# MingSun-Tse/Efficient-NeRF

Hardware: AMD Instinct MI355X
Metric: rays/sec at 800x800 (R2L W256D88) (higher is better)
Workload: dtype f16+bf6 (1 fp16 MFMA pass + both hi/lo correction terms on the block-scaled MFMA in OCP bf6 (e3m2) at 4x the fp16 rate, fp32 accumulate)

## Files before the change

efficient-nerf_amd/csrc/gen/head_gen.py:

```python
#!/usr/bin/env python3
import argparse
import os
import sys

import numpy as np

import isa
from isa import (Ins, State, Filler, vr, ar, vreg, areg, sreg, mfma32_16, mfma32_6, ds_read_b128, ds_read_b64, waitcnt_lgkm,
                 waitcnt_vm, barrier, valu, v_max0, v_accr, v_cvt_pk_f16, v_resid16, v_cvt_pk32_bf6, s_nop, salu, f_to_bf6,
                 pack6, layer_exponent, weight_exps, f32_bits, check_hazards_stream, model_cycles, v_f32_op, v_fma_f32,
                 v_ldexp_f32, v_rndne_f32, v_sin_f32, v_max3_abs)

V_O, V_D, V_X, V_RH, V_RL = 0, 3, 6, 9, 12
V_BQ = 15
V_TT = 16
V_EP = 16
V_VAL = 48
V_EH = 80
V_E6 = 112
V_LO = 136
V_HI = 152
V_A6 = 184
V_L0, V_L1, V_L8A, V_L8B, V_AUX, V_LOFF, V_LANE, V_ST = 196, 197, 198, 199, 200, 201, 202, 203
V_SBA, V_SBL, V_CVA, V_CVL = 204, 205, 206, 207
V_SC = 208
N_VGPR_CLOBBER = 210
V_HMAX = 210
NHI = 8
A_X = 0
N_AGPR_CLOBBER = 128

S_W, S_XOUT, S_WAVE, S_NEG1, S_M0SAVE = 40, 42, 44, 45, 46
S_G = 48
S_WPW = 50
S_C = 51
S_P2 = 54
N_SGPR_LO, N_SGPR_HI = 40, 64

NSLOT = 4
AUX_BYTES = 2048
AUX_SCALES = 1024
NPT = 16
NCH = 2 * NPT


def configure(fmt):
    global FMT, PIECES, CHUNK, PW, LDS_AUX, LDS_BYTES, STREAM_BYTES, ANCH_PER_RT, ANCH_PER_CHUNK, N_ANCH, NHI, NHL, V_HL, V_EL, NAME
    FMT = fmt
    PIECES = 32 if fmt == 'f16' else 28
    CHUNK = PIECES * 1024
    PW = PIECES // 4
    LDS_AUX = NSLOT * CHUNK
    LDS_BYTES = LDS_AUX + AUX_BYTES
    STREAM_BYTES = NCH * CHUNK
    ANCH_PER_RT = 12 if fmt == 'f16' else 6
    ANCH_PER_CHUNK = 4 * ANCH_PER_RT
    N_ANCH = NCH * ANCH_PER_CHUNK
    NHI = 6 if fmt == 'f16' else 8
    NHL, V_HL = 5, 176
    V_EL = 112
    NAME = 'r2l_headx' if fmt == 'f16' else 'r2l_head'


configure('bf6')
EMB_EXP = -1
RES_SHIFT = 12
INV2PI_HI = np.float32(0.15915494)
INV2PI_LO = np.float32(6.4206382e-09)
J_ORDER = [(0, 0), (1, 0)]


def X(u):
    return A_X + u * 16


def EH(b, s):
    return V_EH + b * 16 + s * 4


def E6(b, term):
    return V_E6 + b * 12 + term * 6


def EL(b, s):
    return V_EL + b * 16 + s * 4


def head_col(p, s, h, j):
    if s < 3:
        return (3 * p + s) * 21 + (10 if h else 0) + j
    if j < 6:
        return (3 * p + (j >> 1)) * 21 + (10 if h else 0) + 8 + (j & 1)
    if j == 6:
        return (3 * p + (2 if h else 0)) * 21 + 20
    return -1 if h else (3 * p + 1) * 21 + 20


def piece_hi(k, s):
    return k * 4 + s


def piece_a6(k, t):
    return 16 + k * 2 + t


def piece_a6b(k, t):
    return 24 + k, t * 512


def pack_head(W, b, act_scale=16.0, fmt='bf6'):
    configure(fmt)
    Ws = (W.astype(np.float64) * act_scale).astype(np.float32)
    hi = Ws.astype(np.float16)
    el, ew = weight_exps(layer_exponent(Ws))
    img = np.zeros(STREAM_BYTES, dtype=np.uint8)
    aux = np.zeros(AUX_BYTES // 4, dtype=np.uint32)
    aux[:256] = (b.astype(np.float64) * act_scale).astype(np.float32).view(np.uint32)
    for q in range(4):
        aux[AUX_SCALES // 4 + 4 * q] = 0x01010101 * (127 + el)
        aux[AUX_SCALES // 4 + 4 * q + 1] = 0x01010101 * (127 + ew)
    lanes = np.arange(64)
    h, r = lanes >> 5, lanes & 31
    for p in range(NPT):
        cols = np.array([[[head_col(p, s, hh, j) for j in range(8)] for s in range(4)] for hh in range(2)])
        for u in range(8):
            base = (2 * p + (u >> 2)) * CHUNK
            k = u & 3
            rows = 32 * u + r
            col = cols[h]
            wv = np.where(col >= 0, Ws[rows[:, None, None], np.maximum(col, 0)], 0).astype(np.float32)
            wh = np.where(col >= 0, hi[rows[:, None, None], np.maximum(col, 0)], 0).astype(np.float16)
            for s in range(4):
                o = base + piece_hi(k, s) * 1024
                img[o:o + 1024] = np.ascontiguousarray(wh[:, s, :]).view(np.uint8).reshape(-1)
            if FMT == 'f16':
                wl = (wv.astype(np.float64) - wh.astype(np.float64)).astype(np.float16)
                for s in range(4):
                    o = base + (16 + piece_hi(k, s)) * 1024
                    img[o:o + 1024] = np.ascontiguousarray(wl[:, s, :]).view(np.uint8).reshape(-1)
                continue
            w64, h64 = wv.reshape(64, 32).astype(np.float64), wh.reshape(64, 32).astype(np.float64)
            for t, v in enumerate((np.ldexp(w64 - h64, -el), np.ldexp(w64, -ew))):
                words = pack6(f_to_bf6(v))
                o = base + piece_a6(k, t) * 1024
                img[o:o + 1024] = np.ascontiguousarray(words[:, :4]).view(np.uint8).reshape(-1)
                pc, off = piece_a6b(k, t)
                o = base + pc * 1024 + off
                img[o:o + 512] = np.ascontiguousarray(words[:, 4:]).view(np.uint8).reshape(-1)
    return img, aux.view(np.uint8)


def zop(p):
    return ('s', 'z%d' % p)


def v_sel_half(dst, lo_src, hi_src):
    def emu(st):
        a = isa._f32(st, lo_src).view(np.uint32)
        b = isa._f32(st, hi_src).view(np.uint32)
        st.V[dst] = np.where(np.arange(64) >= 32, b, a)
    return valu('v_cndmask_b32 %s, %s, %s, vcc' % (vreg(dst), isa._opnd(lo_src), isa._opnd(hi_src)), isa._rd(lo_src, hi_src),
                vr(dst), emu)


def dma_piece(i, tag=''):
    voffr = V_L0 if i < 4 else V_LOFF
    imm = 1024 * (i & 3)
    text = 'global_load_lds_dwordx4 %s, %s offset:%d' % (vreg(voffr), sreg(S_G, 2), imm)

    def emu(st):
        copies = []
        g = st.S[S_G]
        for w in range(4):
            dw = (w - st.wave) * PW * 1024
            for l in range(64):
                src = g + int(st.V[voffr][l]) + dw + imm
                dst = st.m0 + dw + imm + l * 16
                assert 0 <= dst and dst + 16 <= LDS_AUX, dst
                assert 0 <= src and src + 16 <= len(st.img), src
                copies.append((dst, st.img[src:src + 16].copy()))
                st.lds_pending[dst:dst + 16] = True
        st.pend_dma.append(copies)
    return Ins(text, 'dma', rd=vr(voffr), emu=emu, cost=8, tag=tag)


def store_group(i, src):
    text = 'global_store_dwordx4 %s, %s, %s offset:%d' % (vreg(V_L0), vreg(src, 4), sreg(S_XOUT, 2), (i & 3) * 1024)

    def emu(st):
        st.xout[i] = st.V[src:src + 4].copy()
    return Ins(text, 'store', rd=vr(V_L0) + vr(src, 4), emu=emu, cost=4)


class HState(State):
    def __init__(self, wave, img, aux, z):
        State.__init__(self, wave, img, np.zeros((1, 1024), dtype=np.uint32), 0, LDS_BYTES)
        self.lds[LDS_AUX:LDS_AUX + len(aux)] = aux
        for p in range(NPT):
            self.S['z%d' % p] = float(z[p])
        self.xout = {}


def embed_ops(p):
    b = p & 1
    ops = []
    for c in range(3):
        ops.append(v_f32_op('mul', V_X + c, zop(p), ('v', V_D + c)))
    for c in range(3):
        ops.append(v_f32_op('add', V_X + c, ('v', V_O + c), ('v', V_X + c)))
    for c in range(3):
        ops.append(v_f32_op('mul', V_RH + c, ('s', S_C), ('v', V_X + c)))
    for c in range(3):
        ops.append(v_fma_f32(V_RL + c, ('v', V_X + c), ('s', S_C), ('v', V_RH + c), neg_c=True))
    for c in range(3):
        ops.append(v_fma_f32(V_RL + c, ('v', V_X + c), ('s', S_C + 1), ('v', V_RL + c)))
    vals = [(8 * c + l, c, l) for c in range(3) for l in range(8)] + [(24 + j, j >> 1, 8 + (j & 1)) for j in range(6)]
    for i0 in range(0, len(vals), 4):
        grp = vals[i0:i0 + 4]
        T = [V_TT + 3 * k for k in range(len(grp))]
        for k, (e, c, l) in enumerate(grp):
            ops.append(v_fma_f32(T[k], ('v', V_RH + c), ('s', S_P2 + l), ('v', V_BQ)))
        for k in range(len(grp)):
            ops.append(v_rndne_f32(T[k] + 1, ('v', T[k])))
        for k in range(len(grp)):
            ops.append(v_f32_op('sub', T[k], ('v', T[k]), ('v', T[k] + 1)))
        for k, (e, c, l) in enumerate(grp):
            ops.append(v_fma_f32(T[k], ('v', V_RL + c), ('s', S_P2 + l), ('v', T[k])))
        for k, (e, c, l) in enumerate(grp):
            ops.append(v_sin_f32(V_VAL + e, ('v', T[k])))
    ops.append(v_sel_half(V_VAL + 30, ('v', V_X + 0), ('v', V_X + 2)))
    ops.append(v_sel_half(V_VAL + 31, ('v', V_X + 1), 0.0))
    for i in range(16):
        ops.append(v_cvt_pk_f16(EH(b, 0) + i, V_VAL + 2 * i, V_VAL + 2 * i + 1))
    for half in range(2):
        for i in range(16):
            ops.append(v_resid16((EL(b, 0) if FMT == 'f16' else V_LO) + i, half, EH(b, 0) + i, half, V_VAL + 2 * i + half, S_NEG1))
    if FMT == 'f16':
        return ops
    ops.append(v_cvt_pk32_bf6(E6(b, 0), EH(b, 0), V_CVA))
    ops.append(v_cvt_pk32_bf6(E6(b, 1), V_LO, V_CVL))
    return ops




def anchor(ci, k, kind, sj):
    if FMT == 'f16':
        return ci * ANCH_PER_CHUNK + k * ANCH_PER_RT + 3 * sj + ('m16', 'mhl', 'mlh').index(kind)
    return ci * ANCH_PER_CHUNK + k * 6 + (sj if kind == 'm16' else 4 + sj)


def lds_addr(slot, byte_off, width):
    off = slot * CHUNK + byte_off
    lo, hi = (V_L0, V_L1) if width == 16 else (V_L8A, V_L8B)
    return (lo, off) if off < 65536 else (hi, off - 65536)


def chunk_issue_seq(cn):
    off = (cn % NCH) * CHUNK
    slot = cn % NSLOT
    seq = [salu('s_add_u32 %s, %s, %s' % (sreg(S_G), sreg(S_W), sreg(S_WPW)), lambda st: st.S.__setitem__(S_G, st.S[S_W] + st.S[S_WPW])),
           salu('s_addc_u32 %s, %s, 0' % (sreg(S_G + 1), sreg(S_W + 1)))]
    if off:
        seq += [salu('s_add_u32 %s, %s, 0x%x' % (sreg(S_G), sreg(S_G), off), lambda st: st.S.__setitem__(S_G, st.S[S_G] + off)),
                salu('s_addc_u32 %s, %s, 0' % (sreg(S_G + 1), sreg(S_G + 1)))]
    seq.append(salu('s_add_u32 m0, %s, 0x%x' % (sreg(S_WPW), slot * CHUNK), lambda st: setattr(st, 'm0', st.S[S_WPW] + slot * CHUNK)))
    seq.append(s_nop(0))
    for i in range(PW):
        if i == 4:
            seq.append(salu('s_add_u32 m0, m0, 0x1000', lambda st: setattr(st, 'm0', st.m0 + 4096)))
            seq.append(s_nop(0))
        seq.append(dma_piece(i, tag=('dma', cn, i)))
    return seq


class Opts:
    def __init__(self, **kw):
        self.rd_lead = 6
        self.rd_lead6 = 5
        self.cap = 7
        self.dma_gap = 1
        self.pair_waits = True
        self.fmt = 'bf6'
        self.__dict__.update(kw)


def build_fillers(opts):
    F = []
    n16, n6 = 0, 0
    last16, last6 = {}, {}
    HALF = ANCH_PER_CHUNK // 2
    for ci in range(NCH):
        for k in range(4):
            for s in range(4):
                a = anchor(ci, k, 'm16', s)
                prev = last16.get(n16 - NHI, -1)
                pc = piece_hi(k, s)
                bv, off = lds_addr(ci % NSLOT, pc * 1024, 16)
                cert = -1 if ci < 3 else (ci - 1) * ANCH_PER_CHUNK + HALF + 1
                F.append(Filler(ds_read_b128(V_HI + (n16 % NHI) * 4, bv, off, tag=('hi', ci, k, s)),
                                max(prev, a - opts.rd_lead, cert), a, ('rd',)))
                last16[n16] = anchor(ci, k, 'mhl', s) if FMT == 'f16' else a
                if FMT == 'f16':
                    al = anchor(ci, k, 'mlh', s)
                    bv, off = lds_addr(ci % NSLOT, (16 + pc) * 1024, 16)
                    F.append(Filler(ds_read_b128(V_HL + (n16 % NHL) * 4, bv, off, tag=('hl', ci, k, s)),
                                    max(last6.get(n16 - NHL, -1), al - opts.rd_lead, cert), al, ('rdl',)))
                    last6[n16] = al
                n16 += 1
            for t in range(2 if FMT != 'f16' else 0):
                a = anchor(ci, k, 'm6', t)
                prev = last6.get(n6 - 2, -1)
                cert = -1 if ci < 3 else (ci - 1) * ANCH_PER_CHUNK + HALF + 1
                e = max(prev, a - opts.rd_lead6, cert)
                bv, off = lds_addr(ci % NSLOT, piece_a6(k, t) * 1024, 16)
                F.append(Filler(ds_read_b128(V_A6 + (n6 & 1) * 6, bv, off, tag=('a6', ci, k, t, 0)), e, a, ('rd6',)))
                pc, po = piece_a6b(k, t)
                bv, off = lds_addr(ci % NSLOT, pc * 1024 + po, 8)
                F.append(Filler(ds_read_b64(V_A6 + (n6 & 1) * 6 + 4, bv, off, tag=('a6', ci, k, t, 1)), e, a, ('rd6',)))
                last6[n6] = a
                n6 += 1
    for p in range(NPT - 1):
        a0, a1 = 2 * p * ANCH_PER_CHUNK, (2 * p + 2) * ANCH_PER_CHUNK
        ops = embed_ops(p + 1)
        for i, ins in enumerate(ops):
            F.append(Filler(ins, a0 + (i * (a1 - a0 - 6)) // len(ops), a1 - 3, ('emb',)))
    for ci in range(NCH):
        ar = ci * ANCH_PER_CHUNK + HALF
        ch = ('dma',)
        F.append(Filler(waitcnt_vm(PW if ci >= 1 else 0), ar - 1, ar + 1, ch))
        F.append(Filler(barrier(), ar - 1, ar + 1, ch))
        k = 0
        for ins in chunk_issue_seq(ci + 3):
            if ins.kind != 'dma' and k == 0:
                F.append(Filler(ins, ar - 1, ar + 3, ch))
            else:
                F.append(Filler(ins, ar + 1 + opts.dma_gap * k, ar + ANCH_PER_CHUNK - 2, ch))
                if ins.kind == 'dma':
                    k += 1
    return F


class Sched:
    def __init__(self):
        self.out = []
        self.ds_issued = 0
        self.ds_done = 0
        self.ds_index = {}

    def emit(self, ins):
        self.out.append(ins)
        if ins.kind == 'ds':
            self.ds_index[ins.tag] = self.ds_issued
            self.ds_issued += 1

    def need(self, key, also=()):
        idx = self.ds_index[key]
        if idx < self.ds_done:
            return
        for k2 in also:
            if k2 in self.ds_index:
                idx = max(idx, self.ds_index[k2])
        self.emit(waitcnt_lgkm(self.ds_issued - idx - 1))
        self.ds_done = idx + 1


def schedule(opts):
    sch = Sched()
    fillers = build_fillers(opts)
    for i, f in enumerate(fillers):
        f.seq = i
    chains = {}
    for f in fillers:
        chains.setdefault(f.chain, []).append(f)
    for ch in chains.values():
        for i in range(len(ch) - 2, -1, -1):
            ch[i].deadline = min(ch[i].deadline, ch[i + 1].deadline)
    heads = {ch: 0 for ch in chains}

    def ready(pos):
        r = []
        for ch, lst in chains.items():
            i = heads[ch]
            if i < len(lst) and lst[i].earliest <= pos:
                r.append(lst[i])
        r.sort(key=lambda f: (f.deadline, f.seq))
        return r

    def issue(f):
        sch.emit(f.ins)
        heads[f.chain] += 1

    while True:
        r = ready(-1)
        if not r:
            break
        issue(r[0])
    n16 = n6 = 0
    for a in range(N_ANCH):
        while True:
            r = [f for f in ready(a - 1) if f.deadline <= a]
            if not r:
                break
            issue(r[0])
        ci, rem = divmod(a, ANCH_PER_CHUNK)
        k, j = divmod(rem, ANCH_PER_RT)
        p, u = ci >> 1, 4 * (ci & 1) + k
        b = p & 1
        if FMT == 'f16':
            sj, which = divmod(j, 3)
            if which == 0:
                sch.need(('hi', ci, k, sj))
                ins = mfma32_16('a', X(u), V_HI + (n16 % NHI) * 4, EH(b, sj), 'a', X(u), tag=('m16', ci, k, sj))
            elif which == 1:
                ins = mfma32_16('a', X(u), V_HI + (n16 % NHI) * 4, EL(b, sj), 'a', X(u), tag=('mhl', ci, k, sj))
            else:
                sch.need(('hl', ci, k, sj))
                ins = mfma32_16('a', X(u), V_HL + (n16 % NHL) * 4, EH(b, sj), 'a', X(u), tag=('mlh', ci, k, sj))
                n16 += 1
        elif j < 4:
            nxt = [('hi', ci, k, j + 1)] if j < 3 and opts.pair_waits else []
            sch.need(('hi', ci, k, j), nxt)
            ins = mfma32_16('a', X(u), V_HI + (n16 % NHI) * 4, EH(b, j), 'a', X(u), tag=('m16', ci, k, j))
            n16 += 1
        else:
            t = j - 4
            sch.need(('a6', ci, k, t, 1))
            ins = mfma32_6('a', X(u), V_A6 + (n6 & 1) * 6, E6(b, t), V_SC + t, V_SBA if t == 0 else V_SBL,
                           tag=('m6', ci, k, t), bfile='v')
            n6 += 1
        sch.emit(ins)
        budget = opts.cap
        while budget > 0:
            r = ready(a)
            if not r:
                break
            issue(r[0])
            budget -= r[0].ins.cost
    while True:
        r = ready(N_ANCH + 10 ** 6)
        if not r:
            break
        issue(r[0])
    return sch.out


def setup_ops():
    L = []
    a = L.append
    a('s_mov_b32 %s, m0' % sreg(S_M0SAVE))
    a('s_mov_b64 %s, %%[wimg]' % sreg(S_W, 2))
    a('s_mov_b64 %s, %%[xout]' % sreg(S_XOUT, 2))
    a('s_mov_b32 %s, %%[wave]' % sreg(S_WAVE))
    a('s_mov_b32 %s, 0xbf800000' % sreg(S_NEG1))
    a('s_mul_i32 %s, %s, 0x%x' % (sreg(S_WPW), sreg(S_WAVE), PW * 1024))
    a('s_mov_b32 %s, 0x%08x' % (sreg(S_C), f32_bits(INV2PI_HI)))
    a('s_mov_b32 %s, 0x%08x' % (sreg(S_C + 1), f32_bits(INV2PI_LO)))
    for l in range(10):
        a('s_mov_b32 %s, 0x%08x' % (sreg(S_P2 + l), f32_bits(2.0 ** l)))
    a('s_mov_b32 vcc_lo, 0')
    a('s_mov_b32 vcc_hi, -1')
    for c in range(3):
        a('v_mov_b32 %s, %%[o%d]' % (vreg(V_O + c), c))
        a('v_mov_b32 %s, %%[d%d]' % (vreg(V_D + c), c))
    a('v_mbcnt_lo_u32_b32 %s, -1, 0' % vreg(V_LANE))
    a('v_mbcnt_hi_u32_b32 %s, -1, %s' % (vreg(V_LANE), vreg(V_LANE)))
    a('v_lshlrev_b32 %s, 4, %s' % (vreg(V_L0), vreg(V_LANE)))
    a('v_add_u32 %s, 0x10000, %s' % (vreg(V_L1), vreg(V_L0)))
    a('v_add_u32 %s, 0x1000, %s' % (vreg(V_LOFF), vreg(V_L0)))
    a('v_lshlrev_b32 %s, 3, %s' % (vreg(V_L8A), vreg(V_LANE)))
    a('v_add_u32 %s, 0x10000, %s' % (vreg(V_L8B), vreg(V_L8A)))
    a('v_lshrrev_b32 %s, 5, %s' % (vreg(V_AUX), vreg(V_LANE)))
    a('v_cvt_f32_u32 %s, %s' % (vreg(V_BQ), vreg(V_AUX)))
    a('v_mul_f32 %s, 0.25, %s' % (vreg(V_BQ), vreg(V_BQ)))
    a('v_lshlrev_b32 %s, 4, %s' % (vreg(V_AUX), vreg(V_AUX)))
    a('v_add_u32 %s, 0x%x, %s' % (vreg(V_AUX), LDS_AUX, vreg(V_AUX)))
    a('v_mov_b32 %s, 0x%08x' % (vreg(V_SBA), 0x01010101 * (127 + EMB_EXP)))
    a('v_mov_b32 %s, 0x%08x' % (vreg(V_SBL), 0x01010101 * (127 + EMB_EXP - RES_SHIFT)))
    a('v_mov_b32 %s, 0x%08x' % (vreg(V_CVA), f32_bits(2.0 ** EMB_EXP)))
    a('v_mov_b32 %s, 0x%08x' % (vreg(V_CVL), f32_bits(2.0 ** (EMB_EXP - RES_SHIFT))))

    def emu(st, o, d):
        lanes = np.arange(64, dtype=np.uint32)
        for c in range(3):
            st.V[V_O + c] = np.asarray(o[c], dtype=np.float32).view(np.uint32)
            st.V[V_D + c] = np.asarray(d[c], dtype=np.float32).view(np.uint32)
        st.V[V_LANE] = lanes
        st.V[V_L0] = lanes * 16
        st.V[V_L1] = lanes * 16 + 65536
        st.V[V_LOFF] = lanes * 16 + 4096
        st.V[V_L8A] = lanes * 8
        st.V[V_L8B] = lanes * 8 + 65536
        st.V[V_BQ] = (0.25 * (lanes >> 5)).astype(np.float32).view(np.uint32)
        st.V[V_AUX] = LDS_AUX + (lanes >> 5) * 16
        st.V[V_SBA] = 0x01010101 * (127 + EMB_EXP)
        st.V[V_SBL] = 0x01010101 * (127 + EMB_EXP - RES_SHIFT)
        st.V[V_CVA] = f32_bits(2.0 ** EMB_EXP)
        st.V[V_CVL] = f32_bits(2.0 ** (EMB_EXP - RES_SHIFT))
        st.S[S_W] = 0
        st.S[S_WPW] = st.wave * PW * 1024
        st.S[S_C] = float(INV2PI_HI)
        st.S[S_C + 1] = float(INV2PI_LO)
        for l in range(10):
            st.S[S_P2 + l] = 2.0 ** l
    return L, emu


def head_ops():
    ops = [waitcnt_vm(0), barrier()]
    for u in range(8):
        for g in range(4):
            ops.append(ds_read_b128(X(u) + 4 * g, V_AUX, 128 * u + 32 * g, tag=('bias', u, g), dfile='a'))
    if FMT != 'f16':
        ops.append(ds_read_b64(V_SC, V_AUX, AUX_SCALES, tag=('scale',)))
    ops += embed_ops(0)
    ops.append(waitcnt_lgkm(0))
    return ops


def tail_ops():
    ops = [s_nop(15), s_nop(15)]
    for i in range(32):
        t = V_EP + (i % 8) * 4
        for r in range(4):
            ops.append(v_accr(t + r, X(i >> 2) + 4 * (i & 3) + r))
        for r in range(4):
            ops.append(v_max0(t + r, t + r))
        for r in (0, 2):
            ops.append(v_max3_abs(V_HMAX, t + r, t + r + 1))
        ops.append(store_group(i, t))
        if i % 4 == 3 and i < 31:
            ops.append(salu('s_add_u32 %s, %s, 0x1000' % (sreg(S_XOUT), sreg(S_XOUT))))
            ops.append(salu('s_addc_u32 %s, %s, 0' % (sreg(S_XOUT + 1), sreg(S_XOUT + 1))))
    ops.append(s_nop(1))
    return ops


def prologue_ops():
    seq = []
    for k in range(3):
        seq += chunk_issue_seq(k)
    return seq


def block_stream(opts):
    configure(opts.fmt)
    return head_ops() + schedule(opts) + tail_ops()


def emit(dirname, opts):
    configure(opts.fmt)
    setup, _ = setup_ops()
    body = block_stream(opts)
    n = {}
    for ins in body:
        n[ins.kind] = n.get(ins.kind, 0) + 1
    with open(os.path.join(dirname, NAME + '_asm.inc'), 'w') as f:
        f.write('// GENERATED by gen/head_gen.py -- do not edit.  Head layer of one 128-ray tile: %s\n' %
                ', '.join('%s %d' % kv for kv in sorted(n.items())))
        for line in setup + [i.text for i in body] + ['s_mov_b32 m0, %s' % sreg(S_M0SAVE)]:
            f.write('"%s\\n\\t"\n' % line)
    with open(os.path.join(dirname, NAME + '_pro_asm.inc'), 'w') as f:
        f.write('// GENERATED by gen/head_gen.py -- do not edit.  Ring prologue: chunks 0..2 of the stream\n')
        pro = ['s_mov_b32 %s, m0' % sreg(S_M0SAVE), 's_mov_b64 %s, %%[wimg]' % sreg(S_W, 2),
               's_mov_b32 %s, %%[wave]' % sreg(S_WAVE), 's_mul_i32 %s, %s, 0x%x' % (sreg(S_WPW), sreg(S_WAVE), PW * 1024),
               'v_mbcnt_lo_u32_b32 %s, -1, 0' % vreg(V_LANE), 'v_mbcnt_hi_u32_b32 %s, -1, %s' % (vreg(V_LANE), vreg(V_LANE)),
               'v_lshlrev_b32 %s, 4, %s' % (vreg(V_L0), vreg(V_LANE)), 'v_add_u32 %s, 0x1000, %s' % (vreg(V_LOFF), vreg(V_L0))]
        for line in pro + [i.text for i in prologue_ops()] + ['s_mov_b32 m0, %s' % sreg(S_M0SAVE)]:
            f.write('"%s\\n\\t"\n' % line)

    def clob(vregs, na):
        regs = ['v%d' % i for i in vregs] + ['a%d' % i for i in range(na)]
        regs += ['s%d' % i for i in range(N_SGPR_LO, N_SGPR_HI)] + ['vcc', 'scc', 'memory']
        return ', '.join('"%s"' % r for r in regs) + '\n'

    with open(os.path.join(dirname, NAME + '_clobbers.inc'), 'w') as f:
        f.write('// GENERATED by gen/head_gen.py: registers the tile block owns\n' + clob(range(N_VGPR_CLOBBER), N_AGPR_CLOBBER))
    with open(os.path.join(dirname, NAME + '_pro_clobbers.inc'), 'w') as f:
        f.write('// GENERATED by gen/head_gen.py: registers the ring prologue owns\n' + clob([V_L0, V_LOFF, V_LANE], 0))
    return n, body


def emulate_tile(opts, img, aux, o, d, z, wave=0, n_tiles=1, check_hazards=True, body=None):
    configure(opts.fmt)
    body = body or block_stream(opts)
    st = HState(wave, img, aux, z)
    _, setup = setup_ops()
    setup(st, o, d)
    st.run(prologue_ops())
    for _ in range(n_tiles):
        st.xout = {}
        st.run(body)
    errs = list(st.errors)
    if st.pend_ds:
        errs.append('%d LDS reads never waited for' % len(st.pend_ds))
    if check_hazards:
        errs += check_hazards_stream(body)
    out = np.stack([st.xout[i] for i in range(32)]).view(np.float32)
    return out, errs


def main():
    ap = argparse.ArgumentParser()
    ap.add_argument('--emit', help='directory for r2l_head_asm.inc / r2l_head_pro_asm.inc')
    ap.add_argument('--dump')
    ap.add_argument('--rd-lead', type=int, default=6)
    ap.add_argument('--rd-lead6', type=int, default=5)
    ap.add_argument('--cap', type=int, default=7)
    ap.add_argument('--dma-gap', type=int, default=1)
    ap.add_argument('--no-pair-waits', action='store_true')
    ap.add_argument('--fmt', default='bf6', choices=['bf6', 'f16'], help='f16: three fp16 passes (r2l_headx_*.inc, R2L_PREC_FP16X3_ASM)')
    a = ap.parse_args()
    opts = Opts(rd_lead=a.rd_lead, rd_lead6=a.rd_lead6, cap=a.cap, dma_gap=a.dma_gap, pair_waits=not a.no_pair_waits, fmt=a.fmt)
    if a.emit:
        n, body = emit(a.emit, opts)
        print('wrote', a.emit, n, 'model cycles per tile', model_cycles(body))
    if a.dump:
        body = block_stream(opts)
        with open(a.dump, 'w') as f:
            for ins in body:
                f.write(ins.text + '\n')
        print('model cycles per tile', model_cycles(body))


if __name__ == '__main__':
    sys.exit(main())
```

efficient-nerf_amd/csrc/r2l_capi.hip:

```cpp
#include <hip/hip_runtime.h>
#include <math.h>
#include <stdarg.h>
#include <stdio.h>
#include <stdlib.h>
#include <string.h>

#include <string>
#include <vector>

#include "../../include/r2l_hip.h"
#include "r2l_common.h"
#include "r2l_kernels.h"
#include "r2l_host_util.h"

static thread_local std::string g_err;

const char* r2l_last_error(void) { return g_err.c_str(); }

int r2l_set_error(int code, const char* fmt, ...) {
    char buf[512];
    va_list ap;
    va_start(ap, fmt);
    vsnprintf(buf, sizeof buf, fmt, ap);
    va_end(ap);
// ... 946 lines not shown
    p.act_out = c->act_out;
    p.block_resid = c->block_resid ? 1.0f : 0.0f;
    p.chunks_per_tile = r2l_chunks_per_tile(c->n_block);
    p.scratch = c->d_scratch;
}

static int timing_events(r2l_ctx* c, hipEvent_t* e0, hipEvent_t* e1) {
    if (c->ev_used + 2 > (int)c->ev.size()) {
        for (int i = 0; i < 2; ++i) {
            hipEvent_t e;
            hipError_t er = hipEventCreate(&e);
            if (er != hipSuccess) return r2l_set_error(R2L_EHIP, "hipEventCreate: %s", hipGetErrorString(er));
            c->ev.push_back(e);
        }
    }
    *e0 = c->ev[c->ev_used];
    *e1 = c->ev[c->ev_used + 1];
    c->ev_used += 2;
    return R2L_OK;
}

static int ensure_x(r2l_ctx* c, int tiles, bool need_xb) {
    auto grow = [&](float** buf, int* cap) -> int {
        if (tiles <= *cap) return R2L_OK;
        if (*buf) (void)hipFree(*buf);
        *buf = nullptr;
        *cap = 0;
        const size_t bytes = (size_t)tiles * R2L_TILE_RAYS * R2L_WIDTH * sizeof(float);
        hipError_t e = hipMalloc((void**)buf, bytes);
        if (e != hipSuccess) return r2l_set_error(R2L_EHIP, "hipMalloc x buffer (%zu B): %s", bytes, hipGetErrorString(e));
        *cap = tiles;
        return R2L_OK;
    };
    int rc = grow(&c->d_xa, &c->x_tiles);
    if (rc == R2L_OK && need_xb) rc = grow(&c->d_xb, &c->xb_tiles);
    return rc;
}

static int launch_split(r2l_ctx* c, const R2LParams& p, hipStream_t s) {
    const int slice = p.n_tiles < R2L_SLICE_TILES ? p.n_tiles : R2L_SLICE_TILES;
    const bool fused_form = c->n_block > 0 && c->use_residual && c->fuse_tail;
    int split = -1;
    if (two_part(c->mode) && c->n_block > 0) {
        split = c->split_block < 0 ? c->n_block / 2 : c->split_block;
        if (split > c->n_block) split = c->n_block;
    }
    const bool two_bodies = split > 0 && split < c->n_block;
    int rc = ensure_x(c, slice, c->n_block > 0 && (!fused_form || two_bodies));
    if (rc) return rc;
    c->last_stream = s;
    for (int t0 = 0; t0 < p.n_tiles; t0 += R2L_SLICE_TILES) {
        const int nt = p.n_tiles - t0 < R2L_SLICE_TILES ? p.n_tiles - t0 : R2L_SLICE_TILES;
        const int grid = balanced_grid(nt, c->n_cu);
        R2LParams ph = p;
        ph.wimg = c->d_img[c->mode];
        ph.xbuf = c->d_xa;
        ph.tile_begin = t0;
        ph.n_tiles = nt;
        ph.range = c->d_range;
        hipError_t e = r2l_launch_head(ph, grid, s, head_x3(c->mode));
        if (e != hipSuccess) return r2l_set_error(R2L_EHIP, "r2l head launch: %s", hipGetErrorString(e));
        const float* body_out = c->d_xa;
        bool fused = false;
        if (c->n_block > 0 && c->calib_pending && scaled_mode(c->mode)) {
            e = r2l_launch_calib(c->d_xa, c->d_wcal, c->n_block, nt, c->act_scale, c->d_stats, c->d_body + c->aux_off,
                                 c->d_exps, c->calib_started, s);
            c->calib_started = 1;
            if (nt >= R2L_CALIB_TILES || ++c->calib_calls >= R2L_CALIB_MAX_CALLS) c->calib_pending = 0;
            if (e != hipSuccess) return r2l_set_error(R2L_EHIP, "r2l calibration launch: %s", hipGetErrorString(e));
        }
        if (c->n_block > 0) {
            R2LBodyParams pb;
            pb.wimg = c->d_body;
            pb.aux = c->d_body + c->aux_off;
            pb.xin = c->d_xa;
            pb.n_tiles = nt;
            pb.n_block = c->n_block;
            fused = c->use_residual && c->fuse_tail;
            pb.rgb = fused ? p.rgb : nullptr;
            pb.xout = fused ? c->d_xa : c->d_xb;
            pb.tail = reinterpret_cast<const float*>(c->d_body + c->tail_off);
            pb.n_rays = p.n_rays;
            pb.tile_begin = t0;
            pb.e4m3 = e4m3_terms(c->mode) ? 1 : c->mode == R2L_PREC_FP16X3_ASM ? 2 : 0;
            R2LBodyParams p2 = pb;
            if (split >= 0) {
                const int n3 = split, n6 = c->n_block - split;
                R2LBodyParams& q6 = two_bodies ? p2 : pb;
                if (two_bodies) {
                    pb.rgb = nullptr;
                    pb.xout = c->d_xb;
                    p2.xin = c->d_xb;
                }
                if (n3 > 0) {
                    pb.wimg = c->d_body2;
                    pb.aux = c->d_body2 + c->aux_off2;
                    pb.tail = reinterpret_cast<const float*>(c->d_body2 + c->tail_off2);
                    pb.e4m3 = 2;
                    pb.n_block = n3;
                }
                if (n6 > 0) {
                    q6.wimg = c->d_body + (size_t)split * 16 * (e4m3_terms(c->mode) ? R2L_BODY8_CHUNK : R2L_BF6_CHUNK);
                    q6.aux = c->d_body + c->aux_off;
                    q6.tail = reinterpret_cast<const float*>(c->d_body + c->tail_off);
                    q6.e4m3 = e4m3_terms(c->mode) ? 1 : 0;
                    q6.n_block = n6;
                    if (split > 0) {
                        q6.aux = c->d_body2 + c->aux_split_off;
                        e = r2l_launch_split_aux(c->d_body + c->aux_off, split, n6, c->d_body2 + c->aux_split_off, s);
                        if (e != hipSuccess) return r2l_set_error(R2L_EHIP, "r2l split aux launch: %s", hipGetErrorString(e));
                    }
                }
            }
// ... 162 lines not shown
```

efficient-nerf_amd/csrc/r2l_kernels.hip:

```cpp
#include <hip/hip_runtime.h>
#include <stdint.h>

#include <atomic>

#include "../../include/r2l_hip.h"
#include "r2l_common.h"
#include "r2l_kernels.h"

#include "r2l_device.h"

struct Ray6 {
    float ox, oy, oz, dx, dy, dz;
    __device__ __forceinline__ float o(int k) const { return k == 0 ? ox : (k == 1 ? oy : oz); }
    __device__ __forceinline__ float d(int k) const { return k == 0 ? dx : (k == 1 ? dy : dz); }
};

__device__ __forceinline__ Ray6 make_ray(const R2LParams& p, int ray) {
    Ray6 r;
    if (p.rays_o != nullptr) {
        const float* po = p.rays_o + (size_t)ray * 3;
        const float* pd = p.rays_d + (size_t)ray * 3;
        r.ox = po[0]; r.oy = po[1]; r.oz = po[2];
        r.dx = pd[0]; r.dy = pd[1]; r.dz = pd[2];
        return r;
// ... 358 lines not shown
template <int NP, bool GA>
static hipError_t launch_resmlp_ga(const R2LParams& p, int grid, hipStream_t stream) {
    static std::atomic<bool> attr_set[64];
    int dev = 0;
    hipError_t e = hipGetDevice(&dev);
    if (e != hipSuccess) return e;
    if (dev < 0 || dev >= 64 || !attr_set[dev]) {
        e = hipFuncSetAttribute(reinterpret_cast<const void*>(&r2l_resmlp_kernel<NP, GA>),
                                hipFuncAttributeMaxDynamicSharedMemorySize, KCfg<NP>::LDS);
        if (e != hipSuccess) return e;
        if (dev >= 0 && dev < 64) attr_set[dev] = true;
    }
    hipLaunchKernelGGL((r2l_resmlp_kernel<NP, GA>), dim3(grid), dim3(256), KCfg<NP>::LDS, stream, p);
    return hipGetLastError();
}
template <int NP>
static hipError_t launch_resmlp(const R2LParams& p, int grid, hipStream_t stream) {
    if (p.act_head == 0.0f && p.act_in == 0.0f && p.act_out == 1.0f && p.block_resid == 1.0f) return launch_resmlp_ga<NP, false>(p, grid, stream);
    return launch_resmlp_ga<NP, true>(p, grid, stream);
}

template <bool X3>
__global__ __launch_bounds__(256, 1) void r2l_head_kernel(R2LParams p) {
    extern __shared__ __attribute__((aligned(16))) char r2l_head_lds[];
    const int wave = __builtin_amdgcn_readfirstlane(threadIdx.x >> 6);
    const int lane = threadIdx.x & 63;
    {
        const uint4* src = reinterpret_cast<const uint4*>(p.wimg + (X3 ? R2L_HEADX_STREAM_BYTES : R2L_HEAD_STREAM_BYTES));
        uint4* dst = reinterpret_cast<uint4*>(r2l_head_lds + 4 * (X3 ? R2L_HEADX_CHUNK : 28672));
        if (threadIdx.x < R2L_HEAD_AUX_BYTES / 16) dst[threadIdx.x] = src[threadIdx.x];
    }
    __syncthreads();
    if constexpr (X3) {
        asm volatile(
#include "r2l_headx_pro_asm.inc"
            :
            : [wimg] "s"(p.wimg), [wave] "s"(wave)
            :
#include "r2l_headx_pro_clobbers.inc"
        );
    } else {
        asm volatile(
#include "r2l_head_pro_asm.inc"
            :
            : [wimg] "s"(p.wimg), [wave] "s"(wave)
            :
#include "r2l_head_pro_clobbers.inc"
        );
    }
    const __attribute__((address_space(4))) float* zc = (const __attribute__((address_space(4))) float*)p.z;
    const float z0 = zc[0], z1 = zc[1], z2 = zc[2], z3 = zc[3], z4 = zc[4], z5 = zc[5], z6 = zc[6], z7 = zc[7], z8 = zc[8],
                z9 = zc[9], z10 = zc[10], z11 = zc[11], z12 = zc[12], z13 = zc[13], z14 = zc[14], z15 = zc[15];
    register float hmax asm("v210") = 0.0f;
    for (int tile = blockIdx.x; tile < p.n_tiles; tile += gridDim.x) {
        const int ray_raw = (p.tile_begin + tile) * R2L_TILE_RAYS + wave * R2L_RAYS_PER_WAVE + (lane & 31);
        const Ray6 r = make_ray(p, ray_raw < p.n_rays ? ray_raw : p.n_rays - 1);
        float* xout = p.xbuf + ((size_t)(tile * R2L_WAVES + wave) * 32) * 256;
#define R2L_HEAD_BLOCK_OPERANDS                                                                                          \
            : [hmax] "+v"(hmax)                                                                                          \
            : [wimg] "s"(p.wimg), [wave] "s"(wave), [xout] "s"(xout), [o0] "v"(r.ox), [o1] "v"(r.oy), [o2] "v"(r.oz),     \
              [d0] "v"(r.dx), [d1] "v"(r.dy), [d2] "v"(r.dz), [z0] "s"(z0), [z1] "s"(z1), [z2] "s"(z2), [z3] "s"(z3),    \
              [z4] "s"(z4), [z5] "s"(z5), [z6] "s"(z6), [z7] "s"(z7), [z8] "s"(z8), [z9] "s"(z9), [z10] "s"(z10),        \
              [z11] "s"(z11), [z12] "s"(z12), [z13] "s"(z13), [z14] "s"(z14), [z15] "s"(z15)
        if constexpr (X3) {
            asm volatile(
#include "r2l_headx_asm.inc"
                R2L_HEAD_BLOCK_OPERANDS
                :
#include "r2l_headx_clobbers.inc"
            );
        } else {
            asm volatile(
#include "r2l_head_asm.inc"
                R2L_HEAD_BLOCK_OPERANDS
                :
#include "r2l_head_clobbers.inc"
            );
        }
#undef R2L_HEAD_BLOCK_OPERANDS
    }
    asm volatile("s_waitcnt vmcnt(0)" ::: "memory");
    if (p.range != nullptr) {
        float m = hmax;
#pragma unroll
        for (int k = 32; k >= 1; k >>= 1) m = fmaxf(m, __shfl_xor(m, k));
        if (lane == 0 && m > 0.0f) atomicMax(p.range, __float_as_uint(m));
    }
}

hipError_t r2l_launch_head(const R2LParams& p, int grid, hipStream_t stream, int x3) {
    static std::atomic<bool> attr_set[64];
    int dev = 0;
    hipError_t e = hipGetDevice(&dev);
    if (e != hipSuccess) return e;
    if (dev < 0 || dev >= 64 || !attr_set[dev]) {
        e = hipFuncSetAttribute(reinterpret_cast<const void*>(&r2l_head_kernel<false>), hipFuncAttributeMaxDynamicSharedMemorySize,
                                R2L_HEAD_LDS);
        if (e == hipSuccess)
            e = hipFuncSetAttribute(reinterpret_cast<const void*>(&r2l_head_kernel<true>), hipFuncAttributeMaxDynamicSharedMemorySize,
                                    R2L_HEADX_LDS);
        if (e != hipSuccess) return e;
        if (dev >= 0 && dev < 64) attr_set[dev] = true;
    }
    if (x3) hipLaunchKernelGGL(r2l_head_kernel<true>, dim3(grid), dim3(256), R2L_HEADX_LDS, stream, p);
    else hipLaunchKernelGGL(r2l_head_kernel<false>, dim3(grid), dim3(256), R2L_HEAD_LDS, stream, p);
    return hipGetLastError();
}
// ... 20 lines not shown
```

Baseline: 62.40 million.

## Process two ray tiles per pass of the head weight stream

Adds a paired build of the bf6 head kernel in which each pass of the streamed weights through LDS feeds MFMAs for two 128-ray tiles. Each weight chunk is fetched once for twice the rays, which is meant to halve DMA and LDS-read traffic per tile, and the head launch grid is halved to match. In exchange it needs a remapped register layout that uses nearly all VGPRs and AGPRs, may lower occupancy, and handles an odd leftover tile with the single-tile path. A diagnostic 'knock' option is also added to measure how much streaming half the weights is worth.

```diff
diff --git a/efficient-nerf_amd/csrc/gen/head_gen.py b/efficient-nerf_amd/csrc/gen/head_gen.py
--- a/efficient-nerf_amd/csrc/gen/head_gen.py
+++ b/efficient-nerf_amd/csrc/gen/head_gen.py
@@ -37,6 +37,26 @@
 S_P2 = 54
 N_SGPR_LO, N_SGPR_HI = 40, 64
 
+_MAP_NAMES = ('V_O', 'V_D', 'V_X', 'V_RH', 'V_RL', 'V_BQ', 'V_TT', 'V_EP', 'V_VAL', 'V_EH', 'V_E6', 'V_LO', 'V_HI', 'V_A6', 'V_L0', 'V_L1',
+              'V_L8A', 'V_L8B', 'V_AUX', 'V_LOFF', 'V_LANE', 'V_SBA', 'V_SBL', 'V_CVA', 'V_CVL', 'V_SC', 'N_AGPR_CLOBBER')
+_MAP_TILE = {k: globals()[k] for k in _MAP_NAMES}
+_MAP_PAIR = dict(V_O=0, V_D=3,
+                 V_X=12, V_RH=15, V_RL=18, V_BQ=21,
+                 V_TT=22,
+                 V_EP=22,
+                 V_VAL=34,
+                 V_EH=66,
+                 V_E6=130,
+                 V_LO=178,
+                 V_A6=194,
+                 V_L0=206, V_L1=207, V_SC=208,
+                 V_L8A=211, V_L8B=212, V_AUX=213, V_LOFF=214, V_LANE=215, V_SBA=216, V_SBL=217, V_CVA=218, V_CVL=219,
+                 V_HI=220,
+                 N_AGPR_CLOBBER=256)
+PAIR_VGPR_CLOBBER = [r for r in range(12, 252) if r != V_HMAX]
+PAIR = False
+NT = 1
+
 NSLOT = 4
 AUX_BYTES = 2048
 AUX_SCALES = 1024
@@ -44,7 +64,11 @@
 NCH = 2 * NPT
 
 
-def configure(fmt):
+def configure(fmt, pair=False):
+    global PAIR, NT
+    assert not (pair and fmt != 'bf6'), 'the pair build exists for the bf6 head only'
+    PAIR, NT = pair, 2 if pair else 1
+    globals().update(_MAP_PAIR if pair else _MAP_TILE)
     global FMT, PIECES, CHUNK, PW, LDS_AUX, LDS_BYTES, STREAM_BYTES, ANCH_PER_RT, ANCH_PER_CHUNK, N_ANCH, NHI, NHL, V_HL, V_EL, NAME
     FMT = fmt
     PIECES = 32 if fmt == 'f16' else 28
@@ -59,7 +83,7 @@
     NHI = 6 if fmt == 'f16' else 8
     NHL, V_HL = 5, 176
     V_EL = 112
-    NAME = 'r2l_headx' if fmt == 'f16' else 'r2l_head'
+    NAME = 'r2l_headx' if fmt == 'f16' else 'r2l_head2' if pair else 'r2l_head'
 
 
 configure('bf6')
@@ -70,16 +94,16 @@
 J_ORDER = [(0, 0), (1, 0)]
 
 
-def X(u):
-    return A_X + u * 16
-
-
-def EH(b, s):
-    return V_EH + b * 16 + s * 4
-
-
-def E6(b, term):
-    return V_E6 + b * 12 + term * 6
+def X(u, t=0):
+    return A_X + t * 128 + u * 16
+
+
+def EH(b, s, t=0):
+    return V_EH + t * 32 + b * 16 + s * 4
+
+
+def E6(b, term, t=0):
+    return V_E6 + t * 24 + b * 12 + term * 6
 
 
 def EL(b, s):
@@ -184,11 +208,11 @@
     return Ins(text, 'dma', rd=vr(voffr), emu=emu, cost=8, tag=tag)
 
 
-def store_group(i, src):
+def store_group(i, src, t=0):
     text = 'global_store_dwordx4 %s, %s, %s offset:%d' % (vreg(V_L0), vreg(src, 4), sreg(S_XOUT, 2), (i & 3) * 1024)
 
     def emu(st):
-        st.xout[i] = st.V[src:src + 4].copy()
+        st.xout[32 * t + i] = st.V[src:src + 4].copy()
     return Ins(text, 'store', rd=vr(V_L0) + vr(src, 4), emu=emu, cost=4)
 
 
@@ -201,13 +225,13 @@
         self.xout = {}
 
 
-def embed_ops(p):
+def embed_ops(p, t=0):
     b = p & 1
     ops = []
     for c in range(3):
-        ops.append(v_f32_op('mul', V_X + c, zop(p), ('v', V_D + c)))
+        ops.append(v_f32_op('mul', V_X + c, zop(p), ('v', V_D + 6 * t + c)))
     for c in range(3):
-        ops.append(v_f32_op('add', V_X + c, ('v', V_O + c), ('v', V_X + c)))
+        ops.append(v_f32_op('add', V_X + c, ('v', V_O + 6 * t + c), ('v', V_X + c)))
     for c in range(3):
         ops.append(v_f32_op('mul', V_RH + c, ('s', S_C), ('v', V_X + c)))
     for c in range(3):
@@ -231,14 +255,14 @@
     ops.append(v_sel_half(V_VAL + 30, ('v', V_X + 0), ('v', V_X + 2)))
     ops.append(v_sel_half(V_VAL + 31, ('v', V_X + 1), 0.0))
     for i in range(16):
-        ops.append(v_cvt_pk_f16(EH(b, 0) + i, V_VAL + 2 * i, V_VAL + 2 * i + 1))
+        ops.append(v_cvt_pk_f16(EH(b, 0, t) + i, V_VAL + 2 * i, V_VAL + 2 * i + 1))
     for half in range(2):
         for i in range(16):
-            ops.append(v_resid16((EL(b, 0) if FMT == 'f16' else V_LO) + i, half, EH(b, 0) + i, half, V_VAL + 2 * i + half, S_NEG1))
+            ops.append(v_resid16((EL(b, 0) if FMT == 'f16' else V_LO) + i, half, EH(b, 0, t) + i, half, V_VAL + 2 * i + half, S_NEG1))
     if FMT == 'f16':
         return ops
-    ops.append(v_cvt_pk32_bf6(E6(b, 0), EH(b, 0), V_CVA))
-    ops.append(v_cvt_pk32_bf6(E6(b, 1), V_LO, V_CVL))
+    ops.append(v_cvt_pk32_bf6(E6(b, 0, t), EH(b, 0, t), V_CVA))
+    ops.append(v_cvt_pk32_bf6(E6(b, 1, t), V_LO, V_CVL))
     return ops
 
 
@@ -282,6 +306,8 @@
         self.dma_gap = 1
         self.pair_waits = True
         self.fmt = 'bf6'
+        self.pair = False
+        self.knock = False
         self.__dict__.update(kw)
 
 
@@ -291,6 +317,8 @@
     last16, last6 = {}, {}
     HALF = ANCH_PER_CHUNK // 2
     for ci in range(NCH):
+        if opts.knock and ci & 1:
+            continue
         for k in range(4):
             for s in range(4):
                 a = anchor(ci, k, 'm16', s)
@@ -322,7 +350,7 @@
                 n6 += 1
     for p in range(NPT - 1):
         a0, a1 = 2 * p * ANCH_PER_CHUNK, (2 * p + 2) * ANCH_PER_CHUNK
-        ops = embed_ops(p + 1)
+        ops = [ins for t in range(NT) for ins in embed_ops(p + 1, t)]
         for i, ins in enumerate(ops):
             F.append(Filler(ins, a0 + (i * (a1 - a0 - 6)) // len(ops), a1 - 3, ('emb',)))
     for ci in range(NCH):
@@ -332,6 +360,8 @@
         F.append(Filler(barrier(), ar - 1, ar + 1, ch))
         k = 0
         for ins in chunk_issue_seq(ci + 3):
+            if opts.knock and ins.kind == 'dma' and not ci & 1:
+                continue
             if ins.kind != 'dma' and k == 0:
                 F.append(Filler(ins, ar - 1, ar + 3, ch))
             else:
@@ -342,8 +372,9 @@
 
 
 class Sched:
-    def __init__(self):
+    def __init__(self, knock=False):
         self.out = []
+        self.knock = knock
         self.ds_issued = 0
         self.ds_done = 0
         self.ds_index = {}
@@ -355,6 +386,8 @@
             self.ds_issued += 1
 
     def need(self, key, also=()):
+        if self.knock and key not in self.ds_index:
+            return
         idx = self.ds_index[key]
         if idx < self.ds_done:
             return
@@ -366,7 +399,7 @@
 
 
 def schedule(opts):
-    sch = Sched()
+    sch = Sched(opts.knock)
     fillers = build_fillers(opts)
     for i, f in enumerate(fillers):
         f.seq = i
@@ -421,22 +454,24 @@
         elif j < 4:
             nxt = [('hi', ci, k, j + 1)] if j < 3 and opts.pair_waits else []
             sch.need(('hi', ci, k, j), nxt)
-            ins = mfma32_16('a', X(u), V_HI + (n16 % NHI) * 4, EH(b, j), 'a', X(u), tag=('m16', ci, k, j))
+            ins = [mfma32_16('a', X(u, rt), V_HI + (n16 % NHI) * 4, EH(b, j, rt), 'a', X(u, rt), tag=('m16', ci, k, j) + (rt,) * PAIR)
+                   for rt in range(NT)]
             n16 += 1
         else:
             t = j - 4
             sch.need(('a6', ci, k, t, 1))
-            ins = mfma32_6('a', X(u), V_A6 + (n6 & 1) * 6, E6(b, t), V_SC + t, V_SBA if t == 0 else V_SBL,
-                           tag=('m6', ci, k, t), bfile='v')
+            ins = [mfma32_6('a', X(u, rt), V_A6 + (n6 & 1) * 6, E6(b, t, rt), V_SC + t, V_SBA if t == 0 else V_SBL,
+                            tag=('m6', ci, k, t) + (rt,) * PAIR, bfile='v') for rt in range(NT)]
             n6 += 1
-        sch.emit(ins)
-        budget = opts.cap
-        while budget > 0:
-            r = ready(a)
-            if not r:
-                break
-            issue(r[0])
-            budget -= r[0].ins.cost
+        for rt, mf in enumerate(ins if isinstance(ins, list) else [ins]):
+            sch.emit(mf)
+            budget = opts.cap
+            while budget > 0:
+                r = ready(a if rt == NT - 1 else a - 1)
+                if not r:
+                    break
+                issue(r[0])
+                budget -= r[0].ins.cost
     while True:
         r = ready(N_ANCH + 10 ** 6)
         if not r:
@@ -460,7 +495,7 @@
         a('s_mov_b32 %s, 0x%08x' % (sreg(S_P2 + l), f32_bits(2.0 ** l)))
     a('s_mov_b32 vcc_lo, 0')
     a('s_mov_b32 vcc_hi, -1')
-    for c in range(3):
+    for c in range(3 if not PAIR else 0):
         a('v_mov_b32 %s, %%[o%d]' % (vreg(V_O + c), c))
         a('v_mov_b32 %s, %%[d%d]' % (vreg(V_D + c), c))
     a('v_mbcnt_lo_u32_b32 %s, -1, 0' % vreg(V_LANE))
@@ -482,9 +517,10 @@
 
     def emu(st, o, d):
         lanes = np.arange(64, dtype=np.uint32)
-        for c in range(3):
-            st.V[V_O + c] = np.asarray(o[c], dtype=np.float32).view(np.uint32)
-            st.V[V_D + c] = np.asarray(d[c], dtype=np.float32).view(np.uint32)
+        for t, (ot, dt) in enumerate(zip(o, d) if PAIR else [(o, d)]):
+            for c in range(3):
+                st.V[V_O + 6 * t + c] = np.asarray(ot[c], dtype=np.float32).view(np.uint32)
+                st.V[V_D + 6 * t + c] = np.asarray(dt[c], dtype=np.float32).view(np.uint32)
         st.V[V_LANE] = lanes
         st.V[V_L0] = lanes * 16
         st.V[V_L1] = lanes * 16 + 65536
@@ -508,30 +544,34 @@
 
 def head_ops():
     ops = [waitcnt_vm(0), barrier()]
-    for u in range(8):
-        for g in range(4):
-            ops.append(ds_read_b128(X(u) + 4 * g, V_AUX, 128 * u + 32 * g, tag=('bias', u, g), dfile='a'))
+    for t in range(NT):
+        for u in range(8):
+            for g in range(4):
+                ops.append(ds_read_b128(X(u, t) + 4 * g, V_AUX, 128 * u + 32 * g, tag=('bias', u, g) + (t,) * PAIR, dfile='a'))
     if FMT != 'f16':
         ops.append(ds_read_b64(V_SC, V_AUX, AUX_SCALES, tag=('scale',)))
-    ops += embed_ops(0)
+    for t in range(NT):
+        ops += embed_ops(0, t)
     ops.append(waitcnt_lgkm(0))
     return ops
 
 
 def tail_ops():
     ops = [s_nop(15), s_nop(15)]
-    for i in range(32):
-        t = V_EP + (i % 8) * 4
-        for r in range(4):
-            ops.append(v_accr(t + r, X(i >> 2) + 4 * (i & 3) + r))
-        for r in range(4):
-            ops.append(v_max0(t + r, t + r))
-        for r in (0, 2):
-            ops.append(v_max3_abs(V_HMAX, t + r, t + r + 1))
-        ops.append(store_group(i, t))
-        if i % 4 == 3 and i < 31:
-            ops.append(salu('s_add_u32 %s, %s, 0x1000' % (sreg(S_XOUT), sreg(S_XOUT))))
-            ops.append(salu('s_addc_u32 %s, %s, 0' % (sreg(S_XOUT + 1), sreg(S_XOUT + 1))))
+    for rt in range(NT):
+        for i in range(32):
+            t = V_EP + (i % 8) * 4
+            for r in range(4):
+                ops.append(v_accr(t + r, X(i >> 2, rt) + 4 * (i & 3) + r))
+            for r in range(4):
+                ops.append(v_max0(t + r, t + r))
+            for r in (0, 2):
+                ops.append(v_max3_abs(V_HMAX, t + r, t + r + 1))
+            ops.append(store_group(i, t, rt))
+            step = 0x1000 if i < 31 else 0x20000 - 0x7000 if rt < NT - 1 else 0
+            if i % 4 == 3 and step:
+                ops.append(salu('s_add_u32 %s, %s, 0x%x' % (sreg(S_XOUT), sreg(S_XOUT), step)))
+                ops.append(salu('s_addc_u32 %s, %s, 0' % (sreg(S_XOUT + 1), sreg(S_XOUT + 1))))
     ops.append(s_nop(1))
     return ops
 
@@ -544,22 +584,34 @@
 
 
 def block_stream(opts):
-    configure(opts.fmt)
+    configure(opts.fmt, opts.pair)
     return head_ops() + schedule(opts) + tail_ops()
 
 
 def emit(dirname, opts):
-    configure(opts.fmt)
+    configure(opts.fmt, opts.pair)
     setup, _ = setup_ops()
     body = block_stream(opts)
     n = {}
     for ins in body:
         n[ins.kind] = n.get(ins.kind, 0) + 1
     with open(os.path.join(dirname, NAME + '_asm.inc'), 'w') as f:
-        f.write('// GENERATED by gen/head_gen.py -- do not edit.  Head layer of one 128-ray tile: %s\n' %
-                ', '.join('%s %d' % kv for kv in sorted(n.items())))
+        f.write('// GENERATED by gen/head_gen.py -- do not edit.  Head layer of %s: %s\n' %
+                ('two 128-ray tiles on one pass of the weight stream' if PAIR else 'one 128-ray tile',
+                 ', '.join('%s %d' % kv for kv in sorted(n.items()))))
         for line in setup + [i.text for i in body] + ['s_mov_b32 m0, %s' % sreg(S_M0SAVE)]:
             f.write('"%s\\n\\t"\n' % line)
+
+    def clob(vregs, na):
+        regs = ['v%d' % i for i in vregs] + ['a%d' % i for i in range(na)]
+        regs += ['s%d' % i for i in range(N_SGPR_LO, N_SGPR_HI)] + ['vcc', 'scc', 'memory']
+        return ', '.join('"%s"' % r for r in regs) + '\n'
+
+    if PAIR:
+        with open(os.path.join(dirname, NAME + '_clobbers.inc'), 'w') as f:
+            f.write('// GENERATED by gen/head_gen.py: registers the pair block owns (v0-v11 are its read-only operands)\n' +
+                    clob(PAIR_VGPR_CLOBBER, N_AGPR_CLOBBER))
+        return n, body
     with open(os.path.join(dirname, NAME + '_pro_asm.inc'), 'w') as f:
         f.write('// GENERATED by gen/head_gen.py -- do not edit.  Ring prologue: chunks 0..2 of the stream\n')
         pro = ['s_mov_b32 %s, m0' % sreg(S_M0SAVE), 's_mov_b64 %s, %%[wimg]' % sreg(S_W, 2),
@@ -568,11 +620,6 @@
                'v_lshlrev_b32 %s, 4, %s' % (vreg(V_L0), vreg(V_LANE)), 'v_add_u32 %s, 0x1000, %s' % (vreg(V_LOFF), vreg(V_L0))]
         for line in pro + [i.text for i in prologue_ops()] + ['s_mov_b32 m0, %s' % sreg(S_M0SAVE)]:
             f.write('"%s\\n\\t"\n' % line)
-
-    def clob(vregs, na):
-        regs = ['v%d' % i for i in vregs] + ['a%d' % i for i in range(na)]
-        regs += ['s%d' % i for i in range(N_SGPR_LO, N_SGPR_HI)] + ['vcc', 'scc', 'memory']
-        return ', '.join('"%s"' % r for r in regs) + '\n'
 
     with open(os.path.join(dirname, NAME + '_clobbers.inc'), 'w') as f:
         f.write('// GENERATED by gen/head_gen.py: registers the tile block owns\n' + clob(range(N_VGPR_CLOBBER), N_AGPR_CLOBBER))
@@ -600,6 +647,29 @@
     return out, errs
 
 
+def emulate_pair(opts, img, aux, oA, dA, oB, dB, z, wave=0, n_pairs=1, check_hazards=True, body=None):
+    assert opts.pair
+    configure(opts.fmt, True)
+    try:
+        body = body or block_stream(opts)
+        st = HState(wave, img, aux, z)
+        _, setup = setup_ops()
+        setup(st, (oA, oB), (dA, dB))
+        st.run(prologue_ops())
+        for _ in range(n_pairs):
+            st.xout = {}
+            st.run(body)
+        errs = list(st.errors)
+        if st.pend_ds:
+            errs.append('%d LDS reads never waited for' % len(st.pend_ds))
+        if check_hazards:
+            errs += check_hazards_stream(body)
+        out = [np.stack([st.xout[32 * t + i] for i in range(32)]).view(np.float32) for t in range(2)]
+    finally:
+        configure(opts.fmt)
+    return out[0], out[1], errs
+
+
 def main():
     ap = argparse.ArgumentParser()
     ap.add_argument('--emit', help='directory for r2l_head_asm.inc / r2l_head_pro_asm.inc')
@@ -609,18 +679,20 @@
     ap.add_argument('--cap', type=int, default=7)
     ap.add_argument('--dma-gap', type=int, default=1)
     ap.add_argument('--no-pair-waits', action='store_true')
+    ap.add_argument('--pair', action='store_true', help='two ray tiles per pass of the weight stream (r2l_head2_*.inc)')
+    ap.add_argument('--knock', action='store_true', help='diagnostic build with wrong results: what streaming half the weights is worth')
     ap.add_argument('--fmt', default='bf6', choices=['bf6', 'f16'], help='f16: three fp16 passes (r2l_headx_*.inc, R2L_PREC_FP16X3_ASM)')
     a = ap.parse_args()
-    opts = Opts(rd_lead=a.rd_lead, rd_lead6=a.rd_lead6, cap=a.cap, dma_gap=a.dma_gap, pair_waits=not a.no_pair_waits, fmt=a.fmt)
+    opts = Opts(rd_lead=a.rd_lead, rd_lead6=a.rd_lead6, cap=a.cap, dma_gap=a.dma_gap, pair_waits=not a.no_pair_waits, fmt=a.fmt, knock=a.knock, pair=a.pair)
     if a.emit:
         n, body = emit(a.emit, opts)
-        print('wrote', a.emit, n, 'model cycles per tile', model_cycles(body))
+        print('wrote', a.emit, n, 'model cycles per tile', model_cycles(body) // NT)
     if a.dump:
         body = block_stream(opts)
         with open(a.dump, 'w') as f:
             for ins in body:
                 f.write(ins.text + '\n')
-        print('model cycles per tile', model_cycles(body))
+        print('model cycles per tile', model_cycles(body) // NT)
 
 
 if __name__ == '__main__':
diff --git a/efficient-nerf_amd/csrc/r2l_capi.hip b/efficient-nerf_amd/csrc/r2l_capi.hip
--- a/efficient-nerf_amd/csrc/r2l_capi.hip
+++ b/efficient-nerf_amd/csrc/r2l_capi.hip
@@ -1022,13 +1022,14 @@
     for (int t0 = 0; t0 < p.n_tiles; t0 += R2L_SLICE_TILES) {
         const int nt = p.n_tiles - t0 < R2L_SLICE_TILES ? p.n_tiles - t0 : R2L_SLICE_TILES;
         const int grid = balanced_grid(nt, c->n_cu);
+        const int head_grid = head_x3(c->mode) ? grid : balanced_grid((nt + 1) / 2, c->n_cu);
         R2LParams ph = p;
         ph.wimg = c->d_img[c->mode];
         ph.xbuf = c->d_xa;
         ph.tile_begin = t0;
         ph.n_tiles = nt;
         ph.range = c->d_range;
-        hipError_t e = r2l_launch_head(ph, grid, s, head_x3(c->mode));
+        hipError_t e = r2l_launch_head(ph, head_grid, s, head_x3(c->mode));
         if (e != hipSuccess) return r2l_set_error(R2L_EHIP, "r2l head launch: %s", hipGetErrorString(e));
         const float* body_out = c->d_xa;
         bool fused = false;
diff --git a/efficient-nerf_amd/csrc/r2l_kernels.hip b/efficient-nerf_amd/csrc/r2l_kernels.hip
--- a/efficient-nerf_amd/csrc/r2l_kernels.hip
+++ b/efficient-nerf_amd/csrc/r2l_kernels.hip
@@ -434,7 +434,42 @@
     const float z0 = zc[0], z1 = zc[1], z2 = zc[2], z3 = zc[3], z4 = zc[4], z5 = zc[5], z6 = zc[6], z7 = zc[7], z8 = zc[8],
                 z9 = zc[9], z10 = zc[10], z11 = zc[11], z12 = zc[12], z13 = zc[13], z14 = zc[14], z15 = zc[15];
     register float hmax asm("v210") = 0.0f;
-    for (int tile = blockIdx.x; tile < p.n_tiles; tile += gridDim.x) {
+    int tile_first = blockIdx.x, tile_step = gridDim.x;
+    if constexpr (!X3) {
+        const int n_pairs = p.n_tiles >> 1;
+        for (int pr = blockIdx.x; pr < n_pairs; pr += gridDim.x) {
+            const int ray0 = (p.tile_begin + 2 * pr) * R2L_TILE_RAYS + wave * R2L_RAYS_PER_WAVE + (lane & 31);
+            const int ray1 = ray0 + R2L_TILE_RAYS;
+            const Ray6 r0 = make_ray(p, ray0 < p.n_rays ? ray0 : p.n_rays - 1);
+            const Ray6 r1 = make_ray(p, ray1 < p.n_rays ? ray1 : p.n_rays - 1);
+            float* xout = p.xbuf + ((size_t)(2 * pr * R2L_WAVES + wave) * 32) * 256;
+            register float o00 asm("v0") = r0.ox;
+            register float o01 asm("v1") = r0.oy;
+            register float o02 asm("v2") = r0.oz;
+            register float d00 asm("v3") = r0.dx;
+            register float d01 asm("v4") = r0.dy;
+            register float d02 asm("v5") = r0.dz;
+            register float o10 asm("v6") = r1.ox;
+            register float o11 asm("v7") = r1.oy;
+            register float o12 asm("v8") = r1.oz;
+            register float d10 asm("v9") = r1.dx;
+            register float d11 asm("v10") = r1.dy;
+            register float d12 asm("v11") = r1.dz;
+            asm volatile(
+#include "r2l_head2_asm.inc"
+                : [hmax] "+v"(hmax)
+                : [wimg] "s"(p.wimg), [wave] "s"(wave), [xout] "s"(xout), "v"(o00), "v"(o01), "v"(o02), "v"(d00), "v"(d01), "v"(d02),
+                  "v"(o10), "v"(o11), "v"(o12), "v"(d10), "v"(d11), "v"(d12), [z0] "s"(z0), [z1] "s"(z1), [z2] "s"(z2), [z3] "s"(z3),
+                  [z4] "s"(z4), [z5] "s"(z5), [z6] "s"(z6), [z7] "s"(z7), [z8] "s"(z8), [z9] "s"(z9), [z10] "s"(z10),
+                  [z11] "s"(z11), [z12] "s"(z12), [z13] "s"(z13), [z14] "s"(z14), [z15] "s"(z15)
+                :
+#include "r2l_head2_clobbers.inc"
+            );
+        }
+        tile_first = (p.n_tiles & 1) && (int)blockIdx.x == n_pairs % (int)gridDim.x ? p.n_tiles - 1 : p.n_tiles;
+        tile_step = 1;
+    }
+    for (int tile = tile_first; tile < p.n_tiles; tile += tile_step) {
         const int ray_raw = (p.tile_begin + tile) * R2L_TILE_RAYS + wave * R2L_RAYS_PER_WAVE + (lane & 31);
         const Ray6 r = make_ray(p, ray_raw < p.n_rays ? ray_raw : p.n_rays - 1);
         float* xout = p.xbuf + ((size_t)(tile * R2L_WAVES + wave) * 32) * 256;
```

Measured after the change: 62.36 million. About the same (-0.1%).
